# ictnlp/StreamSpeech

Hardware: AMD Instinct MI355X
Metric: real-time factor (RTFx = audio seconds / wall seconds) + utterances/sec, offline S2ST fr-en (higher is better)
Workload: dtype f32

## Files before the change

### include/streamspeech_hip.h

```cpp
#ifndef STREAMSPEECH_HIP_H
#define STREAMSPEECH_HIP_H

#include <stddef.h>
#include <stdint.h>

#ifdef __cplusplus
extern "C" {
#endif

#define SS_ABI_VERSION 2

typedef struct ss_model ss_model;
typedef struct ss_vocoder ss_vocoder;
typedef struct ss_scratch ss_scratch;
typedef struct ss_stream_pool ss_stream_pool;

typedef struct ss_config {
  int32_t input_feat, conv_channels, conv_kernel;
  int32_t enc_dim, enc_ffn, enc_heads, enc_layers, dw_kernel;
  int32_t src_vocab, tgt_vocab;
  int32_t mt_layers, dec_dim, dec_ffn, dec_heads;
  int32_t t2u_layers, unit_layers, unit_vocab, ctc_upsample;
  int32_t pad, eos, unk;
  int32_t max_rel_pos;
// ... 245 lines not shown
                             int64_t* h_n_samples);
int ss_batch_t2u_units_pad(ss_model* m, void* stream, int B, const float* d_feats, int feat_rows, const int32_t* h_n,
                           const int32_t* h_n_tail_pad, int t2u_causal, int mask_eos, int32_t* d_raw, int32_t* d_tokens,
                           int32_t* d_counts);
int ss_batch_mt_features(ss_model* m, void* stream, int B, const float* d_enc_out, const int32_t* h_Tp, const int32_t* h_tokens,
                         const int32_t* h_n_tokens, const int32_t* h_n_tail_pad, float* d_feats, int feat_rows);
int ss_batch_vocoder_tail(ss_vocoder* v, void* stream, int B, const int32_t* d_codes, const int32_t* h_K, const int32_t* h_n_new,
                          const int32_t* h_ctx, const int32_t* h_rf, int dur_prediction, float* d_out, int64_t out_capacity,
                          int32_t* h_win_first, int32_t* h_dur, int64_t* h_out_start, int64_t* h_n_out);

int ss_prof_enable(int cls_mask);
int ss_prof_enable_hi(int cls_mask);
int ss_prof_reset(void);
int ss_prof_read(int cls, double* h_ms_total, double* h_flops_total, int64_t* h_launches,
                 double* h_bytes_total);
int ss_prof_totals(int cls, double* h_flops_total, double* h_bytes_total, int64_t* h_launches);
int ss_prof_read_issued(int cls, double* h_issued_flops_total);
int ss_prof_shape_log(int on);
int ss_prof_shape_dump(char* buf, int cap);
int ss_prof_num_classes(void);
const char* ss_prof_class_name(int cls);

int ss_model_set_pack_invariant(ss_model* m, int on);
int ss_model_get_pack_invariant(ss_model* m);
int ss_debug_canon(int mode);

int ss_debug_last_logits(ss_model* m, void* stream, float* d_out, int64_t cap_floats, int* h_rows, int* h_cols);

int ss_op_ffn_fused(void* stream, const float* dX, int ldx, float* dY, int ldy, const float* ln_g, const float* ln_b,
                    const float* dW1, const float* db1, const float* dW2, const float* db2, float alpha,
                    const float* ln2_g, const float* ln2_b, int M, int D, int F);
int ss_debug_ffn(int grid, int row_tiles_per_wave, int enable);
int ss_debug_rtlin(int grid, int enable);
int ss_debug_conv_c64(int enable);
int ss_debug_conv_c32(int enable);
int ss_debug_conv_c16(int enable);
int64_t ss_debug_enc_step_launches(void);
int ss_op_ln_linear(void* stream, const float* dX, int ldx, const float* ln_g, const float* ln_b, const float* dW,
                    const float* dbias, const float* dR, int ldr, float* dC, int ldc, int M, int N, int K, int act, float alpha,
                    int glu);

int ss_debug_force_tile(int bm, int bn, int ks);
int ss_debug_sk_errors(void);
int ss_debug_attention_split(int v);
int ss_debug_attention_q16(int v);
int ss_debug_enc_step_inject_timeout(ss_model* m);
int ss_debug_scratch_audit(ss_scratch* sc, size_t* booked, size_t* held);
int ss_debug_mt_inject_timeout(ss_model* m);

int ss_op_conv_gemm(void* stream, const float* dA, int lda, const float* dW, const float* dbias,
                    const float* dR, int ldr, const float* dR2, int ldr2, float* dC, int ldc,
                    int M, int N, int Cin, int taps, int dil, int stride, int pad, int in_len,
                    int chunk, int in_act, float in_slope, int act, float alpha, float div, int glu);
int ss_op_conv_f16(void* stream, const float* dA, const float* dW, const float* dbias, const float* dR, const float* dR2,
                   float* dC, float* dC2, int M, int C, int taps, int dil, int in_act, float in_slope, int act, float div,
                   const int32_t* d_segs, int nseg);
int ss_op_layernorm(void* stream, const float* dx, int ldx, float* dy, int ldy, const float* dg,
                    const float* db, int M, int D, float eps);
int ss_op_attention(void* stream, const float* dQ, int ldq, const float* dK, int ldk, const float* dV,
                    int ldv, float* dO, int ldo, int Tq, int Tk, int H, float scale, int causal,
                    int chunk, const float* dP, int ldp, const float* du, const float* dv);
typedef struct ss_op_attn_args {
  const float* Q; const float* K; const float* V; float* O;
  int32_t ldq, ldk, ldv, ldo;
  int32_t Tq, Tk, H;
  float scale;
// ... 30 lines not shown
```

### streamspeech_amd/csrc/debug_ops.hip

```cpp
#include "model_internal.hpp"

extern "C" int ss_op_conv_gemm(void* stream, const float* dA, int lda, const float* dW, const float* dbias,
                               const float* dR, int ldr, const float* dR2, int ldr2, float* dC, int ldc, int M,
                               int N, int Cin, int taps, int dil, int stride, int pad, int in_len, int chunk,
                               int in_act, float in_slope, int act, float alpha, float div, int glu) {
  GemmArgs a;
  a.A = dA; a.lda = lda; a.W = dW; a.bias = dbias; a.R = dR; a.ldr = ldr; a.R2 = dR2; a.ldr2 = ldr2; a.C = dC; a.ldc = ldc;
  a.M = M; a.N = N; a.Cin = Cin; a.taps = taps; a.dil = dil; a.stride = stride; a.pad = pad; a.in_len = in_len;
  a.chunk = chunk; a.in_act = in_act; a.in_slope = in_slope; a.act = act; a.alpha = alpha; a.div = div; a.glu = glu;
  a.same_rows = (stride == 1 && M == in_len) ? 1 : 0;
  static thread_local std::map<hipStream_t, DevBuf> wino_tmps;
  DevBuf& wino_tmp = wino_tmps[(hipStream_t)stream];
  if ((conv_c64w_enabled() && N == 64 && Cin == 64 && taps >= 3 && conv_c64_eligible(a)) ||
      (conv_c128w_enabled() && N == 128 && Cin == 128 && taps >= 3 && a.same_rows && !glu) ||
      (conv_c256w_enabled() && N == 256 && Cin == 256 && taps >= 3 && a.same_rows && !glu) ||
      (conv_c32w_enabled() && N == 32 && Cin == 32 && taps >= 3 && conv_c32_eligible(a))) {
    RET(wino_tmp.ensure((size_t)N * ((taps + 2) / 3) * 4 * N * sizeof(float)));
    RET(launch_wino_pack(dW, wino_tmp.f(), N, taps, (hipStream_t)stream));
    a.Wwino = wino_tmp.f();
  }
  return launch_conv_gemm(a, (hipStream_t)stream);
}

extern "C" int ss_op_conv_f16(void* stream, const float* dA, const float* dW, const float* dbias, const float* dR, const float* dR2,
// ... 45 lines not shown
  return launch_conv_gemm(a, (hipStream_t)stream);
}
extern "C" int ss_debug_conv_c64(int enable) {
  if (enable == 4 || enable == 5) { conv_c64w_debug(enable == 5); return SS_OK; }
  if (enable == 6 || enable == 7) { conv_c128w_debug(enable == 7); return SS_OK; }
  if (enable == 8 || enable == 9) { conv_c256w_debug(enable == 9); return SS_OK; }
  conv_c64_debug(enable);
  return SS_OK;
}
extern "C" int ss_debug_conv_c32(int enable) {
  if (enable == 4 || enable == 5) { conv_c32w_debug(enable == 5); return SS_OK; }
  conv_c32_debug(enable);
  return SS_OK;
}
extern "C" int ss_debug_conv_c16(int enable) { conv_c16_debug(enable); return SS_OK; }
extern "C" int64_t ss_debug_enc_step_launches(void) { return (int64_t)enc_step_launch_count(); }
extern "C" int ss_debug_scratch_audit(ss_scratch* sc, size_t* booked, size_t* held) {
  if (!sc || !booked || !held) return SS_ERR_ARG;
  size_t sum = 0;
  bool foreign = false;
  for (DevBuf* b : sc->all()) {
    sum += b->bytes;
    if (b->acct != &sc->acct) foreign = true;
  }
  *booked = sc->acct.used;
  *held = sum;
  return foreign ? SS_ERR_ARG : SS_OK;
}
extern "C" int ss_debug_rtlin(int grid, int enable) {
  if (grid < 0) return SS_ERR_ARG;
  rtlin_debug(grid, enable);
  return SS_OK;
}
extern "C" int ss_debug_ffn(int grid, int row_tiles_per_wave, int enable) {
  if (grid < 0 || row_tiles_per_wave < -1 || row_tiles_per_wave > 4) return SS_ERR_ARG;
  ffn_fused_debug_grid(grid);
  ffn_fused_debug_rows(row_tiles_per_wave);
  if (enable >= 0) dispatch_edit([enable](Dispatch& d) { d.ffn_fusion = enable ? 1 : 0; });
  return SS_OK;
}

extern "C" int ss_op_layernorm(void* stream, const float* dx, int ldx, float* dy, int ldy, const float* dg,
                               const float* db, int M, int D, float eps) {
  return launch_layernorm(dx, ldx, dy, ldy, dg, db, M, D, eps, (hipStream_t)stream);
}

static int op_attn_bind_split(AttnArgs& a) {
  static void* scratch = nullptr;
  if (!scratch) {
    SS_HIP_CHECK(hipMalloc(&scratch, attention_split_bytes()));
    SS_HIP_CHECK(hipMemset(scratch, 0, attention_split_bytes()));
  }
  attention_bind_split(a, scratch);
  return SS_OK;
}

extern "C" int ss_op_attention(void* stream, const float* dQ, int ldq, const float* dK, int ldk, const float* dV,
                               int ldv, float* dO, int ldo, int Tq, int Tk, int H, float scale, int causal, int chunk,
                               const float* dP, int ldp, const float* du, const float* dv) {
  AttnArgs a;
  a.Q = dQ; a.ldq = ldq; a.K = dK; a.ldk = ldk; a.V = dV; a.ldv = ldv; a.O = dO; a.ldo = ldo;
  a.Tq = Tq; a.Tk = Tk; a.H = H; a.scale = scale; a.causal = causal; a.chunk = chunk;
  a.P = dP; a.ldp = ldp; a.bias_u = du; a.bias_v = dv;
  if (dP) RET(op_attn_bind_split(a));
  return launch_attention(a, (hipStream_t)stream);
}
// ... 70 lines not shown
```

### streamspeech_amd/csrc/dispatch.hpp

```cpp
#pragma once
#include <functional>

namespace ss {

struct Dispatch {
  int attn_no_mfma = 0;
  int attn_q16 = 1;
  int attn_split = 0;
  int c16_off = 0, c32_off = 0, c64_off = 0;
  long long c16_min_rows = 131072, c32_min_rows = 65536, c64_min_rows = 32768;
  int c64w_on = 1, c128w_on = 1, c256w_on = 1, c32w_on = 1;
  int c64w_min_k = 3;
  long long c128w_min_rows = 65536, c256w_min_rows = 32768;
  int sk_groups = 0;
  int ffn_force_g = 0;
  int ffn_wm = 3, ffn_wm_forced = 0;
  int ffn_fusion = 1;
  int ffn_min_rows = 1000;
  int force_bm = 0, force_bn = 0, force_ks = 0;
  double sk_min_flops = 4e9;
  int no_resblock_fusion = 0, no_pair_fusion = 0;
  int rt_off = 0, rt_min_rows = 193, rt_force_g = 0;
  long long rt_min_units = 4000;
  long long rt_kb_min_units = 256;
  int rt_kb_xmap = 1;
  int rt_kb_uw = 0;
};

const Dispatch& disp();
void dispatch_edit(const std::function<void(Dispatch&)>& fn);

struct CtxDispatch {
  Dispatch d;
  unsigned gen = 0xffffffffu;
  const Dispatch* refresh();
};
struct DispatchScope {
  explicit DispatchScope(const Dispatch* d);
  ~DispatchScope();
  const Dispatch* prev;
};

}
```

### streamspeech_amd/csrc/gemm.hip

```cpp
#include "gemm.hpp"

#include <atomic>
#include <cstdio>
#include <cstdlib>
#include <cstring>
#include <map>
#include <string>
#include <mutex>
#include <tuple>
#include <type_traits>
#include <utility>
#include <vector>

namespace ss {

using f32x4 = __attribute__((ext_vector_type(4))) float;

template <int BM, int BN, int BK, int WM, int WN, int KS, int PD, bool BLK = false>
__global__ __launch_bounds__(256 * KS) void conv_gemm_kernel(const GemmArgs p) {
  static_assert(WM * WN == 4, "4 waves per k-group");
  static_assert(!BLK || KS == 1, "the blocked chain is the KS = 1 form");
  constexpr int LDK = BK + 8;
  constexpr int WTM = BM / WM, WTN = BN / WN;
  constexpr int TM = WTM / 16, TN = WTN / 16;
  static_assert(TM >= 1 && TN >= 1, "wave tile must hold a 16x16 MFMA tile");
  constexpr int KQ = BK / 4;
  constexpr int A_F4 = BM * KQ, W_F4 = BN * KQ;
  constexpr int NA = (A_F4 + 255) / 256, NW = (W_F4 + 255) / 256;
  constexpr int STAGE = (BM + BN) * LDK;
  extern __shared__ __attribute__((aligned(16))) float smem_all[];
  const int kg = threadIdx.x >> 8;
  float* smem = smem_all + kg * 2 * STAGE;

  const int t = threadIdx.x & 255, lane = t & 63, wave = t >> 6;
  const int wm = wave / WN, wn = wave % WN;
  const int r = lane & 15, g = lane >> 4;

  int out_start = 0, out_len = p.M, in_start = 0, in_len = p.in_len, m_begin = p.m_begin, chunk = p.chunk;
  const float* A = p.A;
  if (p.nseg > 0) {
    const int* s = p.segs + 4 * blockIdx.z;
    out_start = s[0]; out_len = s[1]; in_start = s[2]; in_len = s[3];
    if (p.seg_mb) { m_begin = p.seg_mb[2 * blockIdx.z]; chunk = p.seg_mb[2 * blockIdx.z + 1]; }
    if (p.seg_A) A = p.seg_A[blockIdx.z];
  }
  const int m0 = blockIdx.x * BM + m_begin;
  if (m0 >= out_len) return;
  const int n0 = blockIdx.y * BN;
  const int kpt = p.Cin / BK;
// ... 265 lines not shown
          if (p.C2) p.C2[row * p.ldc2 + n + e] = x > 0.f ? x : x * p.c2_slope;
        }
      }
    }
  }
}


template <int SK, int WN, bool LNORM, bool GLU = false>
__global__ __launch_bounds__(256) void smallm_gemm_kernel(const GemmArgs p) {
  static_assert(SK * WN == 4, "4 waves");
  static_assert(!GLU || (SK == 2 && WN == 2), "GLU: wave column 0 = the 16 value columns, 1 = the 16 gate columns of a 32-column block");
  __shared__ f32x4 red[SK > 1 ? (SK - 1) * WN * 64 : 1];
  __shared__ float ln_stat[32];
  const int t = threadIdx.x, lane = t & 63, wave = t >> 6;
  const int sk = wave / WN, wn = wave % WN;
  const int r = lane & 15, g = lane >> 4;
  if ((int)blockIdx.x * (16 * WN) >= p.N) return;
  const int m0 = blockIdx.y * 16;
  const int n0 = blockIdx.x * (16 * WN) + wn * 16;
  const int K = p.Cin;
  const int KC = K / 16;
  const int c_begin = (KC * sk) / SK, c_end = (KC * (sk + 1)) / SK;

  const int am = m0 + r;
  const bool a_ok = am < p.M;
  const float* arow = p.A + (size_t)(a_ok ? am : 0) * p.lda + 4 * g;
  const int wnr = n0 + r;
  const bool w_ok = wnr < p.N;
  const float* wrow = p.W + (size_t)(w_ok ? wnr : 0) * K + 4 * g;

  float mean = 0.f, rstd = 1.f;
  if (LNORM) {
    const int lr = t >> 4, part = t & 15;
    const bool ok = (m0 + lr) < p.M;
    const float* xr = p.A + (size_t)(ok ? m0 + lr : 0) * p.lda + part * 4;
    f32x4 v[8];
    float sm = 0.f;
#pragma unroll
    for (int j = 0; j < 8; ++j) {
      v[j] = f32x4{0.f, 0.f, 0.f, 0.f};
      if (j * 64 < K && ok) v[j] = *reinterpret_cast<const f32x4*>(xr + j * 64);
      sm += (v[j][0] + v[j][1]) + (v[j][2] + v[j][3]);
    }
#pragma unroll
    for (int o = 1; o < 16; o <<= 1) sm += __shfl_xor(sm, o, 64);
    const float mu = sm / (float)K;
    float q = 0.f;
#pragma unroll
    for (int j = 0; j < 8; ++j)
      if (j * 64 < K) {
#pragma unroll
        for (int e = 0; e < 4; ++e) { const float d = v[j][e] - mu; q += d * d; }
      }
#pragma unroll
    for (int o = 1; o < 16; o <<= 1) q += __shfl_xor(q, o, 64);
    if (part == 0) { ln_stat[lr] = mu; ln_stat[16 + lr] = 1.0f / sqrtf(q / (float)K + 1e-5f); }
    __syncthreads();
    mean = ln_stat[r];
    rstd = ln_stat[16 + r];
  }

  f32x4 acc = {0.f, 0.f, 0.f, 0.f}, acc2 = {0.f, 0.f, 0.f, 0.f};
  f32x4 tot = {0.f, 0.f, 0.f, 0.f};
  const bool blocked = (c_end - c_begin) > 8;
  auto load4 = [&](f32x4 (&a)[4], f32x4 (&w)[4], int c) {
#pragma unroll
    for (int u = 0; u < 4; ++u) {
      a[u] = f32x4{0.f, 0.f, 0.f, 0.f};
      w[u] = f32x4{0.f, 0.f, 0.f, 0.f};
      if (a_ok) a[u] = *reinterpret_cast<const f32x4*>(arow + (c + u) * 16);
      if (w_ok) w[u] = *reinterpret_cast<const f32x4*>(wrow + (c + u) * 16);
    }
  };
  auto mma = [&](f32x4 a, f32x4 w, int c) {
    if (LNORM) {
      const f32x4 gm = *reinterpret_cast<const f32x4*>(p.ln_g + c * 16 + 4 * g);
      const f32x4 bt = *reinterpret_cast<const f32x4*>(p.ln_b + c * 16 + 4 * g);
#pragma unroll
      for (int e = 0; e < 4; ++e) a[e] = a_ok ? (a[e] - mean) * rstd * gm[e] + bt[e] : 0.f;
    }
    acc = __builtin_amdgcn_mfma_f32_16x16x4f32(a[0], w[0], acc, 0, 0, 0);
    acc2 = __builtin_amdgcn_mfma_f32_16x16x4f32(a[1], w[1], acc2, 0, 0, 0);
    acc = __builtin_amdgcn_mfma_f32_16x16x4f32(a[2], w[2], acc, 0, 0, 0);
    acc2 = __builtin_amdgcn_mfma_f32_16x16x4f32(a[3], w[3], acc2, 0, 0, 0);
    if (blocked && (c & 3) == 3) {
#pragma unroll
      for (int e = 0; e < 4; ++e) { tot[e] += acc[e] + acc2[e]; acc[e] = 0.f; acc2[e] = 0.f; }
    }
  };
  auto mma4 = [&](f32x4 (&a)[4], f32x4 (&w)[4], int c) {
#pragma unroll
    for (int u = 0; u < 4; ++u) mma(a[u], w[u], c + u);
  };
  const int G = (c_end - c_begin) / 4;
  f32x4 a0[4], w0[4], a1[4], w1[4];
  if (G > 0) load4(a0, w0, c_begin);
  for (int gi = 0; gi < G; gi += 2) {
    const int c = c_begin + 4 * gi;
    if (gi + 1 < G) load4(a1, w1, c + 4);
    mma4(a0, w0, c);
    if (gi + 1 < G) {
      if (gi + 2 < G) load4(a0, w0, c + 8);
      mma4(a1, w1, c + 4);
    }
  }
  for (int c = c_begin + 4 * G; c < c_end; ++c) {
    f32x4 a = {0.f, 0.f, 0.f, 0.f}, w = {0.f, 0.f, 0.f, 0.f};
    if (a_ok) a = *reinterpret_cast<const f32x4*>(arow + c * 16);
    if (w_ok) w = *reinterpret_cast<const f32x4*>(wrow + c * 16);
    mma(a, w, c);
  }
#pragma unroll
  for (int e = 0; e < 4; ++e) acc[e] = tot[e] + (acc[e] + acc2[e]);

  if (SK > 1) {
    if (sk > 0) red[((sk - 1) * WN + wn) * 64 + lane] = acc;
    __syncthreads();
    if (!GLU && sk > 0) return;
    if (sk == 0) {
#pragma unroll
      for (int s2 = 1; s2 < SK; ++s2) {
        const f32x4 o = red[((s2 - 1) * WN + wn) * 64 + lane];
#pragma unroll
        for (int e = 0; e < 4; ++e) acc[e] += o[e];
      }
    }
  }
  if constexpr (GLU) {
    __shared__ f32x4 gate_tile[64];
    const int ncol = n0 + r;
    const float bcol = (p.bias && ncol < p.N) ? p.bias[ncol] : 0.f;
    if (sk == 0 && wn == 1) {
      f32x4 gt;
#pragma unroll
      for (int e = 0; e < 4; ++e) gt[e] = acc[e] + bcol;
      gate_tile[lane] = gt;
    }
    __syncthreads();
    if (sk != 0 || wn != 0 || ncol + 16 >= p.N) return;
    const f32x4 gt = gate_tile[lane];
    const int oc = (int)blockIdx.x * 16 + r;
#pragma unroll
    for (int e = 0; e < 4; ++e) {
      const int m = m0 + g * 4 + e;
      if (m < p.M) p.C[(size_t)m * p.ldc + oc] = (acc[e] + bcol) * (1.0f / (1.0f + expf(-gt[e])));
    }
    return;
  }
  const int n = n0 + r;
  if (n >= p.N) return;
  const float b = p.bias ? p.bias[n] : 0.f;
#pragma unroll
  for (int e = 0; e < 4; ++e) {
    const int m = m0 + g * 4 + e;
    if (m < p.M) {
      float v = acc[e] + b;
      switch (p.act) {
        case ACT_SILU: v = v / (1.0f + expf(-v)); break;
        case ACT_RELU: v = fmaxf(v, 0.f); break;
        default: break;
      }
      v *= p.alpha;
      if (p.R) v += p.R[(size_t)m * p.ldr + n];
      p.C[(size_t)m * p.ldc + n] = v;
    }
  }
}


template <int MR, int KS, bool LNORM>
__global__ __launch_bounds__(256) void gemv_kernel(const GemmArgs p) {
  constexpr int WPB = 4;
  constexpr int CPB = WPB / KS;
  __shared__ float part[WPB][MR];
  const int t = threadIdx.x, lane = t & 63, wave = t >> 6;
  const int col = blockIdx.x * CPB + wave / KS;
  const int ks = wave % KS;
  const int K = p.Cin;
  const int kper = K / KS;
  const int k0 = ks * kper;
  const int nit = kper / 256;
  const bool col_ok = col < p.N;

  f32x4 wv[8];
  const float* wrow = p.W + (size_t)(col_ok ? col : 0) * K + k0 + 4 * lane;
#pragma unroll
  for (int it = 0; it < 8; ++it) {
    wv[it] = f32x4{0.f, 0.f, 0.f, 0.f};
    if (it < nit && col_ok) wv[it] = *reinterpret_cast<const f32x4*>(wrow + it * 256);
  }
  float acc[MR];
#pragma unroll
  for (int m = 0; m < MR; ++m) {
    acc[m] = 0.f;
    if (m >= p.M) continue;
    const float* xrow = p.A + (size_t)m * p.lda;
    float mean = 0.f, rstd = 1.f;
    if (LNORM) {
      f32x4 xv[8];
// ... 275 lines not shown
}
void sk_workspace_free(SkWorkspace* w) {
  if (!w) return;
  {
    std::lock_guard<std::mutex> lk(g_skw_mu);
    for (size_t i = 0; i < g_skw_live.size(); ++i)
      if (g_skw_live[i] == w) { g_skw_live.erase(g_skw_live.begin() + i); break; }
  }
  if (w->ws) (void)hipFree(w->ws);
  if (w->sync1) (void)hipFree(w->sync1);
  if (w->sync2) (void)hipFree(w->sync2);
  if (w->sync3) (void)hipFree(w->sync3);
  if (w->dbg) (void)hipFree(w->dbg);
  delete w;
}
namespace {
std::mutex g_disp_mu;
std::atomic<unsigned> g_disp_gen{1};
Dispatch env_defaults() {
  Dispatch d;
  auto I = [](const char* k, int dflt) { const char* e = getenv(k); return e ? atoi(e) : dflt; };
  auto L = [](const char* k, long long dflt) { const char* e = getenv(k); return e ? atoll(e) : dflt; };
  d.attn_split = I("SS_ATTN_NO_SPLIT", 0) ? -1 : 0; d.attn_q16 = I("SS_ATTN_Q16", d.attn_q16);
  d.c16_off = I("SS_NO_CONV_C16", 0) ? 1 : 0; d.c32_off = I("SS_NO_CONV_C32", 0) ? 1 : 0; d.c64_off = I("SS_NO_CONV_C64", 0) ? 1 : 0;
  d.c16_min_rows = L("SS_CONV_C16_MIN_ROWS", d.c16_min_rows); d.c32_min_rows = L("SS_CONV_C32_MIN_ROWS", d.c32_min_rows);
  d.c64_min_rows = L("SS_CONV_C64_MIN_ROWS", d.c64_min_rows);
  d.c64w_on = I("SS_CONV_C64_WINOGRAD", 1); d.c128w_on = I("SS_CONV_C128_WINOGRAD", 1); d.c256w_on = I("SS_CONV_C256_WINOGRAD", 1);
  d.c32w_on = I("SS_CONV_C32_WINOGRAD", 1); d.c64w_min_k = I("SS_CONV_C64_WINOGRAD_MIN_K", 3);
  d.c128w_min_rows = L("SS_CONV_C128_MIN_ROWS", d.c128w_min_rows); d.c256w_min_rows = L("SS_CONV_C256_MIN_ROWS", d.c256w_min_rows);
  if (getenv("SS_FFN_WM")) { d.ffn_wm = I("SS_FFN_WM", 3); d.ffn_wm_forced = 1; }
  d.ffn_fusion = I("SS_NO_FFN_FUSION", 0) ? 0 : 1; d.ffn_min_rows = I("SS_FFN_MIN_ROWS", d.ffn_min_rows);
  if (getenv("SS_SK_MIN_GFLOP")) d.sk_min_flops = 1e9 * atof(getenv("SS_SK_MIN_GFLOP"));
  d.no_resblock_fusion = I("SS_NO_RESBLOCK_FUSION", 0); d.no_pair_fusion = I("SS_NO_PAIR_FUSION", 0);
  d.rt_off = I("SS_NO_RTLIN", 0) ? 1 : 0; d.rt_min_rows = I("SS_RTLIN_MIN_ROWS", d.rt_min_rows); d.rt_min_units = L("SS_RTLIN_MIN_UNITS", d.rt_min_units);
  d.rt_kb_min_units = L("SS_RTLIN_KB_MIN_UNITS", d.rt_kb_min_units); d.rt_kb_uw = I("SS_RTLIN_KB_UW", d.rt_kb_uw); d.rt_kb_xmap = I("SS_RTLIN_KB_XMAP", d.rt_kb_xmap);
  return d;
}
Dispatch& process_settings() { static Dispatch d = env_defaults(); return d; }
thread_local const Dispatch* t_disp = nullptr;
thread_local CtxDispatch t_disp_own;
}
void dispatch_edit(const std::function<void(Dispatch&)>& fn) {
  std::lock_guard<std::mutex> lk(g_disp_mu);
  fn(process_settings());
  g_disp_gen.fetch_add(1, std::memory_order_release);
}
const Dispatch* CtxDispatch::refresh() {
  const unsigned now = g_disp_gen.load(std::memory_order_acquire);
  if (gen != now) {
    std::lock_guard<std::mutex> lk(g_disp_mu);
    d = process_settings();
    gen = g_disp_gen.load(std::memory_order_relaxed);
  }
  return &d;
}
const Dispatch& disp() { return t_disp ? *t_disp : *t_disp_own.refresh(); }
DispatchScope::DispatchScope(const Dispatch* d) : prev(t_disp) { t_disp = d; }
DispatchScope::~DispatchScope() { t_disp = prev; }

SkScope::SkScope(SkWorkspace* w) : prev(t_skw), prev_disp(t_disp) { t_skw = w; t_disp = w ? w->disp.refresh() : nullptr; }
SkScope::~SkScope() { t_skw = prev; t_disp = prev_disp; }

int sk_workspace_acquire(hipStream_t stream, SkWorkspace** out) {
  *out = nullptr;
  int dev = 0;
  SS_HIP_CHECK(hipGetDevice(&dev));
// ... 58 lines not shown
    for (unsigned* sy : {w->sync1, w->sync2}) {
      unsigned v = 0;
      if (sy && hipMemcpy(&v, sy + 8, sizeof(v), hipMemcpyDeviceToHost) == hipSuccess) total += (int)v;
    }
  return total;
}

void debug_force_tile(int bm, int bn, int ks) {
  dispatch_edit([=](Dispatch& d) { d.force_bm = bm; d.force_bn = bn; d.force_ks = ks; d.sk_groups = (bm == 1 && bn == 8); });
}
bool debug_tile_forced() { return disp().force_bm != 0; }

static thread_local int t_canon = CANON_NONE;
CanonScope::CanonScope(int mode) : prev(t_canon) { t_canon = mode; }
CanonScope::~CanonScope() { t_canon = prev; }
int canon_mode() { return t_canon; }
void canon_debug_set(int mode) { t_canon = mode; }

static bool smallm_shape_ok(const GemmArgs& a) {
  const bool glu_ok = !a.glu || (a.N % 32 == 0 && a.act == ACT_NONE && a.alpha == 1.f && !a.R);
  return a.taps == 1 && a.stride == 1 && a.pad == 0 && glu_ok && a.nseg == 0 && a.chunk == 0 && a.in_act == ACT_NONE && !a.R2 &&
         !a.C2 && a.div == 0.f && !a.ln_out && (a.act == ACT_NONE || a.act == ACT_SILU || a.act == ACT_RELU) && a.M > 0 &&
         a.M <= 1024 && a.Cin % 64 == 0 && (a.lda & 3) == 0 && (!a.ln_g || a.Cin <= 512);
}

static int launch_canon(const GemmArgs& a, hipStream_t stream) {
  const int M = a.nseg > 0 ? a.max_seg_out : a.M;
  const bool k32 = (a.Cin % 32) == 0;
  const int nseg = a.nseg > 0 ? a.nseg : 1;
  if (a.ln_out) return SS_ERR_ARG;
  if (a.canon == CANON_SMALLM) {
    if (!smallm_shape_ok(a)) return SS_ERR_ARG;
    if (a.glu) return launch_smallm<2, 2, true>(a, stream, PROF_SMALLM_2x2);
    if (a.Cin >= 1024 || a.N <= 4096) return launch_smallm<4, 1>(a, stream, PROF_SMALLM_4x1);
    return launch_smallm<2, 2>(a, stream, PROF_SMALLM_2x2);
  }
  if (a.seg_mb || a.seg_A) {
    if (a.nseg <= 0 || a.ln_g) return SS_ERR_ARG;
    return k32 ? launch_cfg<32, 64, 32, 2, 2, 1, 1, true>(a, stream, PROF_GEMM_32x64x32) : launch_cfg<32, 64, 16, 2, 2, 1, 1, true>(a, stream, PROF_GEMM_32x64x16);
  }
  if (rtlin_shape_ok(a) && (a.ln_g || rtlin_eligible(a))) return launch_rtlin(a, stream);
  if (a.ln_g) return SS_ERR_ARG;
  if (rtlin_kb_eligible(a)) return launch_rtlin_kb(a, stream);
  if (a.N <= 16) return launch_cfg<128, 16, 16, 4, 1, 1, 1, true>(a, stream, PROF_GEMM_128x16x16);
  if (a.N <= 32 && !a.glu) return k32 ? launch_cfg<128, 32, 32, 4, 1, 1, 1, true>(a, stream, PROF_GEMM_128x32x32) : launch_cfg<128, 32, 16, 4, 1, 1, 1, true>(a, stream, PROF_GEMM_128x32x16);
  if (M <= 16) return k32 ? launch_cfg<16, 128, 32, 1, 4, 1, 1, true>(a, stream, PROF_GEMM_16x128x32) : launch_cfg<16, 128, 16, 1, 4, 1, 1, true>(a, stream, PROF_GEMM_16x128x16);
  const long t3264 = (long)cdiv(M, 32) * cdiv(a.N, 64) * nseg;
  if (!k32) return launch_cfg<32, 64, 16, 2, 2, 1, 1, true>(a, stream, PROF_GEMM_32x64x16);
  if (a.glu || t3264 >= 768) return launch_cfg<32, 64, 32, 2, 2, 1, 1, true>(a, stream, PROF_GEMM_32x64x32);
  return launch_cfg<32, 32, 32, 2, 2, 1, 1, true>(a, stream, PROF_GEMM_32x32x32);
}

bool smallm_eligible(const GemmArgs& a) {
  if (disp().force_bm > 1) return false;
  const int M = a.nseg > 0 ? a.max_seg_out : a.M;
  const bool glu_ok = !a.glu || (a.N % 32 == 0 && a.act == ACT_NONE && a.alpha == 1.f && !a.R);
  const bool plain_linear = a.taps == 1 && a.stride == 1 && a.pad == 0 && glu_ok && a.nseg == 0 && a.chunk == 0 &&
                            a.in_act == ACT_NONE && !a.R2 && !a.C2 && a.div == 0.f &&
                            (a.act == ACT_NONE || a.act == ACT_SILU || a.act == ACT_RELU);
  static const int max_rows = getenv("SS_SMALLM_MAX_ROWS") ? atoi(getenv("SS_SMALLM_MAX_ROWS")) : 192;
  return plain_linear && M <= max_rows && M > 0 && a.Cin % 64 == 0 && (a.lda & 3) == 0;
}


int launch_conv_gemm(const GemmArgs& a_in, hipStream_t stream) {
  GemmArgs a = a_in;
// ... 86 lines not shown
```

### streamspeech_amd/csrc/gemm.hpp

```cpp
#pragma once
#include "common.hpp"
#include "dispatch.hpp"

namespace ss {

struct GemmArgs {
  const float* A = nullptr;
  const float* W = nullptr;
  const float* Wwino = nullptr;
  const void* Wf16 = nullptr;
  const float* bias = nullptr;
  const float* R = nullptr;
  const float* R2 = nullptr;
  float* C = nullptr;
  int lda = 0, ldc = 0, ldr = 0, ldr2 = 0;
  int M = 0, N = 0, Cin = 0;
  int taps = 1, dil = 1, stride = 1, pad = 0;
  int in_len = 0;
  int chunk = 0;
  int m_begin = 0;
  int in_act = ACT_NONE;
  float in_slope = 0.1f;
  int act = ACT_NONE;
  float alpha = 1.0f;
// ... 133 lines not shown
void conv_c64_debug(int enable);

bool conv_c32_eligible(const GemmArgs& a);
bool conv_c32_enabled();
int launch_conv_c32(const GemmArgs& a, hipStream_t stream);
void conv_c32_debug(int enable);

bool conv_c16_eligible(const GemmArgs& a);
bool conv_c16_enabled();
int launch_conv_c16(const GemmArgs& a, hipStream_t stream);
void conv_c16_debug(int enable);

bool conv_f16_eligible(const GemmArgs& a);
bool conv_f16_geometry_ok(int C, int taps, int dil);
int launch_conv_f16(const GemmArgs& a, hipStream_t stream);
size_t f16_pack_halves(int C, int taps);
int launch_f16_pack(const float* W, void* Wf, int C, int taps, hipStream_t stream);

bool rtlin_eligible(const GemmArgs& a);
bool rtlin_shape_ok(const GemmArgs& a);
int launch_rtlin(const GemmArgs& a, hipStream_t stream);
void rtlin_debug(int grid, int enable);
bool rtlin_kb_shape_ok(const GemmArgs& a);
bool rtlin_kb_eligible(const GemmArgs& a);
int launch_rtlin_kb(const GemmArgs& a, hipStream_t stream);

bool ffn_fused_eligible(int D, int F, int act, int M, int ldx, int ldy, bool canon = false);
int launch_ffn_fused(const float* X, int ldx, float* Y, int ldy, const float* ln_g, const float* ln_b, const float* W1,
                     const float* b1, const float* W2, const float* b2, float alpha, const float* ln2_g, const float* ln2_b,
                     int M, int D, int F, hipStream_t stream, int canon = 0);
void ffn_fused_debug_grid(int g);
void ffn_fused_debug_rows(int wm);

bool gemv_eligible(const GemmArgs& a);
bool smallm_eligible(const GemmArgs& a);

void debug_force_tile(int bm, int bn, int ks);
bool debug_tile_forced();

int launch_conv_gemm(const GemmArgs& a, hipStream_t stream);

}
```

### streamspeech_amd/lib.py

```python
import ctypes as C
import os

_HERE = os.path.dirname(os.path.abspath(__file__))
LIB_PATH = os.environ.get("SS_HIP_LIB") or os.path.join(_HERE, "libstreamspeech_hip.so")


class SSConfig(C.Structure):
    _fields_ = [(n, C.c_int32) for n in (
        "input_feat", "conv_channels", "conv_kernel", "enc_dim", "enc_ffn", "enc_heads", "enc_layers",
        "dw_kernel", "src_vocab", "tgt_vocab", "mt_layers", "dec_dim", "dec_ffn", "dec_heads",
        "t2u_layers", "unit_layers", "unit_vocab", "ctc_upsample", "pad", "eos", "unk",
        "max_rel_pos", "max_tgt_pos")]


class SSVocoderConfig(C.Structure):
    _fields_ = [
        ("num_embeddings", C.c_int32), ("embedding_dim", C.c_int32), ("model_in_dim", C.c_int32),
        ("upsample_initial_channel", C.c_int32),
        ("n_up", C.c_int32), ("upsample_rates", C.c_int32 * 8), ("upsample_kernel_sizes", C.c_int32 * 8),
        ("n_res", C.c_int32), ("resblock_kernel_sizes", C.c_int32 * 4), ("resblock_dilations", (C.c_int32 * 3) * 4),
        ("dur_hidden", C.c_int32), ("dur_kernel", C.c_int32)]


_vp, _i, _f, _i64 = C.c_void_p, C.c_int, C.c_float, C.c_int64
# ... 128 lines not shown
                                       C.POINTER(_f), C.POINTER(_f), _vp, _i]),
    "ss_batch_mt_beam_continue_plan": (_i, [_i, _i, C.POINTER(C.c_int32), C.POINTER(C.c_int32), C.POINTER(C.c_int32),
                                            C.POINTER(C.c_int32), _i, _i, _i, _i, _i, _i, _i, C.POINTER(C.c_int32),
                                            C.POINTER(C.c_int32), _i64, C.POINTER(_i64)]),
    "ss_batch_fbank_frames": (_i, [_vp, _vp, _i, C.POINTER(_vp), C.POINTER(C.c_int32), C.POINTER(C.c_int32), _f,
                                   C.POINTER(_vp)]),
    "ss_batch_fbank_frames_sr": (_i, [_vp, _vp, _i, C.POINTER(_vp), C.POINTER(C.c_int32), C.POINTER(C.c_int32), C.POINTER(C.c_int32),
                                      C.POINTER(_vp), C.POINTER(C.c_int32), C.POINTER(C.c_int32), C.POINTER(C.c_int32), _f,
                                      C.POINTER(_vp)]),
    "ss_fbank_sr_rows": (_i, [_i64, _i, _i, _i, C.POINTER(C.c_int32), C.POINTER(C.c_int32)]),
    "ss_batch_t2u_units": (_i, [_vp, _vp, _i, _vp, _i, C.POINTER(C.c_int32), _i, _i, _vp, _vp, _vp]),
    "ss_batch_vocoder_forward": (_i, [_vp, _vp, _i, _vp, C.POINTER(C.c_int32), _i, _vp, _vp, _i64, _vp,
                                      C.POINTER(_i64), C.POINTER(_i64)]),
    "ss_batch_t2u_units_pad": (_i, [_vp, _vp, _i, _vp, _i, C.POINTER(C.c_int32), C.POINTER(C.c_int32), _i, _i, _vp, _vp, _vp]),
    "ss_batch_mt_features": (_i, [_vp, _vp, _i, _vp, C.POINTER(C.c_int32), C.POINTER(C.c_int32), C.POINTER(C.c_int32),
                                  C.POINTER(C.c_int32), _vp, _i]),
    "ss_batch_vocoder_tail": (_i, [_vp, _vp, _i, _vp, C.POINTER(C.c_int32), C.POINTER(C.c_int32), C.POINTER(C.c_int32),
                                   C.POINTER(C.c_int32), _i, _vp, _i64, C.POINTER(C.c_int32), C.POINTER(C.c_int32),
                                   C.POINTER(_i64), C.POINTER(_i64)]),
    "ss_prof_enable": (_i, [_i]),
    "ss_prof_enable_hi": (_i, [_i]),
    "ss_prof_reset": (_i, []),
    "ss_prof_read": (_i, [_i, C.POINTER(C.c_double), C.POINTER(C.c_double), C.POINTER(_i64), C.POINTER(C.c_double)]),
    "ss_prof_totals": (_i, [_i, C.POINTER(C.c_double), C.POINTER(C.c_double), C.POINTER(_i64)]),
    "ss_prof_read_issued": (_i, [_i, C.POINTER(C.c_double)]),
    "ss_prof_shape_log": (_i, [_i]),
    "ss_prof_shape_dump": (_i, [C.c_char_p, _i]),
    "ss_prof_num_classes": (_i, []),
    "ss_prof_class_name": (C.c_char_p, [_i]),
    "ss_debug_force_tile": (_i, [_i, _i, _i]),
    "ss_op_ffn_fused": (_i, [_vp, _vp, _i, _vp, _i, _vp, _vp, _vp, _vp, _vp, _vp, _f, _vp, _vp, _i, _i, _i]),
    "ss_debug_ffn": (_i, [_i, _i, _i]),
    "ss_debug_rtlin": (_i, [_i, _i]),
    "ss_debug_conv_c64": (_i, [_i]),
    "ss_debug_conv_c32": (_i, [_i]),
    "ss_debug_conv_c16": (_i, [_i]),
    "ss_debug_enc_step_launches": (_i64, []),
    "ss_debug_scratch_audit": (_i, [_vp, C.POINTER(C.c_size_t), C.POINTER(C.c_size_t)]),
    "ss_op_ln_linear": (_i, [_vp, _vp, _i, _vp, _vp, _vp, _vp, _vp, _i, _vp, _i, _i, _i, _i, _i, _f, _i]),
    "ss_debug_last_logits": (_i, [_vp, _vp, _vp, _i64, C.POINTER(_i), C.POINTER(_i)]),
    "ss_debug_sk_errors": (_i, []),
    "ss_debug_attention_split": (_i, [_i]),
    "ss_debug_attention_q16": (_i, [_i]),
    "ss_op_conv_gemm": (_i, [_vp, _vp, _i, _vp, _vp, _vp, _i, _vp, _i, _vp, _i, _i, _i, _i, _i, _i, _i, _i, _i, _i,
                             _i, _f, _i, _f, _f, _i]),
    "ss_op_conv_f16": (_i, [_vp, _vp, _vp, _vp, _vp, _vp, _vp, _vp, _i, _i, _i, _i, _i, _f, _i, _f, _vp, _i]),
    "ss_op_layernorm": (_i, [_vp, _vp, _i, _vp, _i, _vp, _vp, _i, _i, _f]),
    "ss_op_attention": (_i, [_vp, _vp, _i, _vp, _i, _vp, _i, _vp, _i, _i, _i, _i, _f, _i, _i, _vp, _i, _vp, _vp]),
    "ss_op_attention_ex": (_i, [_vp, C.POINTER(SSOpAttnArgs)]),
    "ss_op_attention_pool": (_i, [_vp, C.POINTER(SSOpPoolAttnArgs)]),
    "ss_debug_attention_no_mfma": (_i, [_i]),
    "ss_op_dwconv_bn_silu": (_i, [_vp, _vp, _i, _vp, _i, _vp, _i, _vp, _vp, _vp, _vp, _f, _i, _i, _i]),
}

_lib = None


SS_ERR_ARG = 2
SS_ERR_CAPACITY = 4
SS_ERR_SCRATCH_CAP = 5
SS_ERR_STREAM_REPEAT = 8


class StreamSpeechHipError(RuntimeError):

    def __init__(self, msg, code=None):
# ... 32 lines not shown
```

Measured before the change: 6339.

## Add multi-tile decode-rows GEMM kernels for small-M linear layers

```diff
diff --git a/include/streamspeech_hip.h b/include/streamspeech_hip.h
--- a/include/streamspeech_hip.h
+++ b/include/streamspeech_hip.h
@@ -301,6 +301,7 @@
                     const float* ln2_g, const float* ln2_b, int M, int D, int F);
 int ss_debug_ffn(int grid, int row_tiles_per_wave, int enable);
 int ss_debug_rtlin(int grid, int enable);
+int ss_debug_decode_rows(int on);
 int ss_debug_conv_c64(int enable);
 int ss_debug_conv_c32(int enable);
 int ss_debug_conv_c16(int enable);
diff --git a/streamspeech_amd/csrc/debug_ops.hip b/streamspeech_amd/csrc/debug_ops.hip
--- a/streamspeech_amd/csrc/debug_ops.hip
+++ b/streamspeech_amd/csrc/debug_ops.hip
@@ -101,6 +101,11 @@
   rtlin_debug(grid, enable);
   return SS_OK;
 }
+extern "C" int ss_debug_decode_rows(int on) {
+  if (!decode_rows_form_ok(on)) return SS_ERR_ARG;
+  decode_rows_debug(on);
+  return SS_OK;
+}
 extern "C" int ss_debug_ffn(int grid, int row_tiles_per_wave, int enable) {
   if (grid < 0 || row_tiles_per_wave < -1 || row_tiles_per_wave > 4) return SS_ERR_ARG;
   ffn_fused_debug_grid(grid);
diff --git a/streamspeech_amd/csrc/decode_rows.hip b/streamspeech_amd/csrc/decode_rows.hip
--- /dev/null
+++ b/streamspeech_amd/csrc/decode_rows.hip
@@ -0,0 +1,281 @@
+#include "gemm.hpp"
+#include "smallm_common.hpp"
+
+namespace ss {
+
+template <int SK, int WN, bool LNORM, int MT, int NT>
+__global__ __launch_bounds__(256) void decode_rows_gemm_kernel(const GemmArgs p) {
+  static_assert(SK * WN == 4, "4 waves");
+  constexpr int TILES = MT * NT;
+  constexpr int CG = (MT + NT) <= 3 ? 4 : 2;
+  __shared__ f32x4 red[SK > 1 ? TILES * 4 * 64 : 1];
+  __shared__ float ln_stat[LNORM ? 32 * MT : 1];
+  const int t = threadIdx.x, lane = t & 63, wave = t >> 6;
+  const int sk = wave / WN, wn = wave % WN;
+  const int r = lane & 15, g = lane >> 4;
+  if ((int)blockIdx.x * (16 * WN * NT) >= p.N) return;
+  const int m0 = blockIdx.y * (16 * MT);
+  const int n0 = blockIdx.x * (16 * WN * NT) + wn * (16 * NT);
+  const int K = p.Cin;
+  const int KC = K / 16;
+  const int c_begin = (KC * sk) / SK, c_end = (KC * (sk + 1)) / SK;
+  const int mt = min(MT, (p.M - m0 + 15) / 16);
+
+  bool a_ok[MT], w_ok[NT];
+  const float* arow[MT];
+  const float* wrow[NT];
+#pragma unroll
+  for (int i = 0; i < MT; ++i) {
+    const int am = m0 + 16 * i + r;
+    a_ok[i] = am < p.M;
+    arow[i] = p.A + (size_t)(a_ok[i] ? am : 0) * p.lda + 4 * g;
+  }
+#pragma unroll
+  for (int j = 0; j < NT; ++j) {
+    const int wnr = n0 + 16 * j + r;
+    w_ok[j] = wnr < p.N;
+    wrow[j] = p.W + (size_t)(w_ok[j] ? wnr : 0) * K + 4 * g;
+  }
+
+  f32x4 acc[MT][NT], acc2[MT][NT], tot[MT][NT];
+#pragma unroll
+  for (int i = 0; i < MT; ++i)
+#pragma unroll
+    for (int j = 0; j < NT; ++j) acc[i][j] = acc2[i][j] = tot[i][j] = f32x4{0.f, 0.f, 0.f, 0.f};
+  const bool blocked = (c_end - c_begin) > 8;
+
+  auto load1 = [&](f32x4 (&a)[MT], f32x4 (&w)[NT], int c) {
+#pragma unroll
+    for (int i = 0; i < MT; ++i) {
+      a[i] = f32x4{0.f, 0.f, 0.f, 0.f};
+      if (i < mt && a_ok[i]) a[i] = *reinterpret_cast<const f32x4*>(arow[i] + c * 16);
+    }
+#pragma unroll
+    for (int j = 0; j < NT; ++j) {
+      w[j] = f32x4{0.f, 0.f, 0.f, 0.f};
+      if (w_ok[j]) w[j] = *reinterpret_cast<const f32x4*>(wrow[j] + c * 16);
+    }
+  };
+  float mean[MT], rstd[MT];
+#pragma unroll
+  for (int i = 0; i < MT; ++i) { mean[i] = 0.f; rstd[i] = 1.f; }
+  auto mma1 = [&](f32x4 (&a)[MT], f32x4 (&w)[NT], int c) {
+    f32x4 gm, bt;
+    if (LNORM) {
+      gm = *reinterpret_cast<const f32x4*>(p.ln_g + c * 16 + 4 * g);
+      bt = *reinterpret_cast<const f32x4*>(p.ln_b + c * 16 + 4 * g);
+    }
+    const bool flush = blocked && (c & 3) == 3;
+#pragma unroll
+    for (int i = 0; i < MT; ++i)
+      if (i < mt) {
+        const f32x4 an = LNORM ? smallm_ln_apply(a[i], a_ok[i], mean[i], rstd[i], gm, bt) : a[i];
+#pragma unroll
+        for (int j = 0; j < NT; ++j) smallm_chunk(an, w[j], acc[i][j], acc2[i][j], tot[i][j], flush);
+      }
+  };
+  auto loadg = [&](f32x4 (&a)[CG][MT], f32x4 (&w)[CG][NT], int c) {
+#pragma unroll
+    for (int u = 0; u < CG; ++u) load1(a[u], w[u], c + u);
+  };
+  auto mmag = [&](f32x4 (&a)[CG][MT], f32x4 (&w)[CG][NT], int c) {
+#pragma unroll
+    for (int u = 0; u < CG; ++u) mma1(a[u], w[u], c + u);
+  };
+  const int G = (c_end - c_begin) / CG;
+  f32x4 a0[CG][MT], w0[CG][NT], a1[CG][MT], w1[CG][NT];
+  if (G > 0) loadg(a0, w0, c_begin);
+  if (G > 1) loadg(a1, w1, c_begin + CG);
+  f32x4 rv[MT][NT];
+#pragma unroll
+  for (int i = 0; i < MT; ++i)
+#pragma unroll
+    for (int j = 0; j < NT; ++j) {
+      rv[i][j] = f32x4{0.f, 0.f, 0.f, 0.f};
+      const int n = n0 + 16 * j + r;
+      if (i < mt && n < p.N && (SK == 1 || (i * NT + j) % SK == sk)) rv[i][j] = smallm_residual(p, m0 + 16 * i + g * 4, n);
+    }
+  if (LNORM) {
+#pragma unroll
+    for (int i = 0; i < MT; ++i)
+      if (i < mt) smallm_ln_stats(p.A, p.lda, m0 + 16 * i, p.M, K, t, ln_stat + 32 * i);
+    __syncthreads();
+#pragma unroll
+    for (int i = 0; i < MT; ++i)
+      if (i < mt) { mean[i] = ln_stat[32 * i + r]; rstd[i] = ln_stat[32 * i + 16 + r]; }
+  }
+  for (int gi = 0; gi < G; gi += 2) {
+    const int c = c_begin + CG * gi;
+    mmag(a0, w0, c);
+    if (gi + 2 < G) loadg(a0, w0, c + 2 * CG);
+    if (gi + 1 < G) {
+      mmag(a1, w1, c + CG);
+      if (gi + 3 < G) loadg(a1, w1, c + 3 * CG);
+    }
+  }
+  if constexpr (CG > 1) {
+    for (int c = c_begin + CG * G; c < c_end; ++c) {
+      load1(a0[0], w0[0], c);
+      mma1(a0[0], w0[0], c);
+    }
+  }
+
+  if (SK > 1) {
+#pragma unroll
+    for (int i = 0; i < MT; ++i)
+#pragma unroll
+      for (int j = 0; j < NT; ++j)
+        if (i < mt) red[((i * NT + j) * 4 + wave) * 64 + lane] = smallm_range_result(acc[i][j], acc2[i][j], tot[i][j]);
+    __syncthreads();
+  }
+#pragma unroll
+  for (int i = 0; i < MT; ++i)
+#pragma unroll
+    for (int j = 0; j < NT; ++j) {
+      if (i >= mt) continue;
+      f32x4 v;
+      if (SK > 1) {
+        if ((i * NT + j) % SK != sk) continue;
+        v = red[((i * NT + j) * 4 + wn) * 64 + lane];
+#pragma unroll
+        for (int s2 = 1; s2 < SK; ++s2) {
+          const f32x4 o = red[((i * NT + j) * 4 + s2 * WN + wn) * 64 + lane];
+#pragma unroll
+          for (int e = 0; e < 4; ++e) v[e] += o[e];
+        }
+      } else {
+        v = smallm_range_result(acc[i][j], acc2[i][j], tot[i][j]);
+      }
+      const int n = n0 + 16 * j + r;
+      if (n < p.N) smallm_epilogue(p, v, m0 + 16 * i + g * 4, n, rv[i][j]);
+    }
+}
+
+constexpr int KB_MAX_BLOCKS = 32;
+template <int KW>
+__global__ __launch_bounds__(256 * KW) void decode_rows_kblock_kernel(const GemmArgs p) {
+  constexpr int SK = 4;
+  __shared__ f32x4 blk[KB_MAX_BLOCKS * 64];
+  const int t = threadIdx.x, lane = t & 63, wave = t >> 6;
+  const int r = lane & 15, g = lane >> 4;
+  if ((int)blockIdx.x * 16 >= p.N) return;
+  const int m0 = blockIdx.y * 16, n0 = blockIdx.x * 16;
+  const int K = p.Cin, KC = K / 16;
+  const int per_wave = KC / (SK * KW);
+  const int c0 = wave * per_wave;
+  const int am = m0 + r, wnr = n0 + r;
+  const bool a_ok = am < p.M, w_ok = wnr < p.N;
+  const float* arow = p.A + (size_t)(a_ok ? am : 0) * p.lda + 4 * g;
+  const float* wrow = p.W + (size_t)(w_ok ? wnr : 0) * K + 4 * g;
+  f32x4 rv = {0.f, 0.f, 0.f, 0.f};
+  for (int cb = 0; cb < per_wave; cb += 8) {
+    f32x4 a[8], w[8];
+#pragma unroll
+    for (int u = 0; u < 8; ++u) {
+      a[u] = f32x4{0.f, 0.f, 0.f, 0.f};
+      w[u] = f32x4{0.f, 0.f, 0.f, 0.f};
+      if (cb + u < per_wave) {
+        if (a_ok) a[u] = *reinterpret_cast<const f32x4*>(arow + (c0 + cb + u) * 16);
+        if (w_ok) w[u] = *reinterpret_cast<const f32x4*>(wrow + (c0 + cb + u) * 16);
+      }
+    }
+    if (cb == 0 && wave == 0 && wnr < p.N) rv = smallm_residual(p, m0 + g * 4, n0 + r);
+#pragma unroll
+    for (int b = 0; b < 2; ++b)
+      if (cb + 4 * b < per_wave) {
+        f32x4 acc = {0.f, 0.f, 0.f, 0.f}, acc2 = {0.f, 0.f, 0.f, 0.f}, s = {0.f, 0.f, 0.f, 0.f};
+#pragma unroll
+        for (int u = 0; u < 4; ++u) smallm_chunk(a[4 * b + u], w[4 * b + u], acc, acc2, s, u == 3);
+        blk[((c0 + cb) / 4 + b) * 64 + lane] = s;
+      }
+  }
+  __syncthreads();
+  if (wave != 0 || wnr >= p.N) return;
+  const int bpr = KC / (4 * SK);
+  f32x4 v;
+  const f32x4 zero = {0.f, 0.f, 0.f, 0.f};
+  for (int sk = 0; sk < SK; ++sk) {
+    f32x4 tot = {0.f, 0.f, 0.f, 0.f};
+    for (int b = 0; b < bpr; ++b) {
+      const f32x4 s = blk[(sk * bpr + b) * 64 + lane];
+#pragma unroll
+      for (int e = 0; e < 4; ++e) tot[e] += s[e];
+    }
+    const f32x4 o = smallm_range_result(zero, zero, tot);
+    if (sk == 0) v = o;
+    else {
+#pragma unroll
+      for (int e = 0; e < 4; ++e) v[e] += o[e];
+    }
+  }
+  smallm_epilogue(p, v, m0 + g * 4, n0 + r, rv);
+}
+
+static bool kblock_ok(const GemmArgs& a, int kw) {
+  const int KC = a.Cin / 16;
+  return !a.ln_g && !a.glu && (a.Cin >= 1024 || a.N <= 4096) &&
+         KC % (16 * kw) == 0 && KC / 4 > 8 && KC / 4 <= KB_MAX_BLOCKS;
+}
+
+template <int KW>
+static int launch_kblock(const GemmArgs& a, hipStream_t stream) {
+  dim3 grid((cdiv(a.N, 16) + 7) & ~7, cdiv(a.M, 16));
+  ProfRec rec{}; bool prof = false;
+  int rc = prof_begin(a, stream, PROF_SMALLM_4x1, rec, prof);
+  if (rc != SS_OK) return rc;
+  hipLaunchKernelGGL((decode_rows_kblock_kernel<KW>), grid, dim3(256 * KW), 0, stream, a);
+  SS_LAUNCH_CHECK();
+  return prof_end(stream, rec, prof);
+}
+
+template <int SK, int WN, int MT, int NT>
+static int launch_form(const GemmArgs& a, hipStream_t stream, ProfCls cls) {
+  dim3 grid((cdiv(a.N, 16 * WN * NT) + 7) & ~7, cdiv(a.M, 16 * MT));
+  ProfRec rec{}; bool prof = false;
+  int rc = prof_begin(a, stream, cls, rec, prof);
+  if (rc != SS_OK) return rc;
+  if (a.ln_g) hipLaunchKernelGGL((decode_rows_gemm_kernel<SK, WN, true, MT, NT>), grid, dim3(256), 0, stream, a);
+  else hipLaunchKernelGGL((decode_rows_gemm_kernel<SK, WN, false, MT, NT>), grid, dim3(256), 0, stream, a);
+  SS_LAUNCH_CHECK();
+  return prof_end(stream, rec, prof);
+}
+
+template <int SK, int WN>
+static int launch_sk(const GemmArgs& a, hipStream_t stream, ProfCls cls, int mt, int nt) {
+  switch (mt * 16 + nt) {
+    case 0x11: return launch_form<SK, WN, 1, 1>(a, stream, cls);
+    case 0x12: return launch_form<SK, WN, 1, 2>(a, stream, cls);
+    case 0x21: return launch_form<SK, WN, 2, 1>(a, stream, cls);
+    case 0x22: return launch_form<SK, WN, 2, 2>(a, stream, cls);
+    case 0x42: return launch_form<SK, WN, 4, 2>(a, stream, cls);
+    default: return SS_ERR_ARG;
+  }
+}
+
+void decode_rows_debug(int on) { dispatch_edit([on](Dispatch& d) { d.decode_rows = on; }); }
+
+bool decode_rows_form_ok(int on) {
+  if (on == 0 || on == 1) return true;
+  const int mt = (on >> 4) & 15, nt = on & 15;
+  if ((on >> 8) == 2) return on == 0x202 || on == 0x204;
+  return (on >> 8) == 1 && ((mt == 1 && (nt == 1 || nt == 2)) || (mt == 2 && (nt == 1 || nt == 2)) || (mt == 4 && nt == 2));
+}
+
+bool decode_rows_takes(const GemmArgs& a) {
+  return disp().decode_rows != 0 && !a.glu && a.M > 16 && (!a.ln_g || a.Cin <= 512);
+}
+
+int launch_decode_rows(const GemmArgs& a, hipStream_t stream) {
+  if (a.glu || a.M <= 0 || a.Cin % 64 != 0 || (a.lda & 3) != 0 || (a.ln_g && a.Cin > 512)) return SS_ERR_ARG;
+  const int on = disp().decode_rows;
+  if ((on >> 8) == 2 && kblock_ok(a, on & 15)) return (on & 15) == 4 ? launch_kblock<4>(a, stream) : launch_kblock<2>(a, stream);
+  if (on == 1 && kblock_ok(a, 4)) return launch_kblock<4>(a, stream);
+  const bool form41 = a.Cin >= 1024 || a.N <= 4096;
+  const long tiles = (long)cdiv(a.M, 16) * cdiv(a.N, form41 ? 16 : 32);
+  int mt = tiles > 800 ? 2 : 1, nt = mt;
+  if ((on >> 8) == 1) { mt = (on >> 4) & 15; nt = on & 15; }
+  if (form41) return launch_sk<4, 1>(a, stream, PROF_SMALLM_4x1, mt, nt);
+  return launch_sk<2, 2>(a, stream, PROF_SMALLM_2x2, mt, nt);
+}
+
+}
diff --git a/streamspeech_amd/csrc/dispatch.hpp b/streamspeech_amd/csrc/dispatch.hpp
--- a/streamspeech_amd/csrc/dispatch.hpp
+++ b/streamspeech_amd/csrc/dispatch.hpp
@@ -19,6 +19,7 @@
   int ffn_min_rows = 1000;
   int force_bm = 0, force_bn = 0, force_ks = 0;
   double sk_min_flops = 4e9;
+  int decode_rows = 1;
   int no_resblock_fusion = 0, no_pair_fusion = 0;
   int rt_off = 0, rt_min_rows = 193, rt_force_g = 0;
   long long rt_min_units = 4000;
diff --git a/streamspeech_amd/csrc/gemm.hip b/streamspeech_amd/csrc/gemm.hip
--- a/streamspeech_amd/csrc/gemm.hip
+++ b/streamspeech_amd/csrc/gemm.hip
@@ -1,4 +1,5 @@
 #include "gemm.hpp"
+#include "smallm_common.hpp"
 
 #include <atomic>
 #include <cstdio>
@@ -13,8 +14,6 @@
 #include <vector>
 
 namespace ss {
-
-using f32x4 = __attribute__((ext_vector_type(4))) float;
 
 template <int BM, int BN, int BK, int WM, int WN, int KS, int PD, bool BLK = false>
 __global__ __launch_bounds__(256 * KS) void conv_gemm_kernel(const GemmArgs p) {
@@ -346,30 +345,7 @@
 
   float mean = 0.f, rstd = 1.f;
   if (LNORM) {
-    const int lr = t >> 4, part = t & 15;
-    const bool ok = (m0 + lr) < p.M;
-    const float* xr = p.A + (size_t)(ok ? m0 + lr : 0) * p.lda + part * 4;
-    f32x4 v[8];
-    float sm = 0.f;
-#pragma unroll
-    for (int j = 0; j < 8; ++j) {
-      v[j] = f32x4{0.f, 0.f, 0.f, 0.f};
-      if (j * 64 < K && ok) v[j] = *reinterpret_cast<const f32x4*>(xr + j * 64);
-      sm += (v[j][0] + v[j][1]) + (v[j][2] + v[j][3]);
-    }
-#pragma unroll
-    for (int o = 1; o < 16; o <<= 1) sm += __shfl_xor(sm, o, 64);
-    const float mu = sm / (float)K;
-    float q = 0.f;
-#pragma unroll
-    for (int j = 0; j < 8; ++j)
-      if (j * 64 < K) {
-#pragma unroll
-        for (int e = 0; e < 4; ++e) { const float d = v[j][e] - mu; q += d * d; }
-      }
-#pragma unroll
-    for (int o = 1; o < 16; o <<= 1) q += __shfl_xor(q, o, 64);
-    if (part == 0) { ln_stat[lr] = mu; ln_stat[16 + lr] = 1.0f / sqrtf(q / (float)K + 1e-5f); }
+    smallm_ln_stats(p.A, p.lda, m0, p.M, K, t, ln_stat);
     __syncthreads();
     mean = ln_stat[r];
     rstd = ln_stat[16 + r];
@@ -391,17 +367,9 @@
     if (LNORM) {
       const f32x4 gm = *reinterpret_cast<const f32x4*>(p.ln_g + c * 16 + 4 * g);
       const f32x4 bt = *reinterpret_cast<const f32x4*>(p.ln_b + c * 16 + 4 * g);
-#pragma unroll
-      for (int e = 0; e < 4; ++e) a[e] = a_ok ? (a[e] - mean) * rstd * gm[e] + bt[e] : 0.f;
-    }
-    acc = __builtin_amdgcn_mfma_f32_16x16x4f32(a[0], w[0], acc, 0, 0, 0);
-    acc2 = __builtin_amdgcn_mfma_f32_16x16x4f32(a[1], w[1], acc2, 0, 0, 0);
-    acc = __builtin_amdgcn_mfma_f32_16x16x4f32(a[2], w[2], acc, 0, 0, 0);
-    acc2 = __builtin_amdgcn_mfma_f32_16x16x4f32(a[3], w[3], acc2, 0, 0, 0);
-    if (blocked && (c & 3) == 3) {
-#pragma unroll
-      for (int e = 0; e < 4; ++e) { tot[e] += acc[e] + acc2[e]; acc[e] = 0.f; acc2[e] = 0.f; }
-    }
+      a = smallm_ln_apply(a, a_ok, mean, rstd, gm, bt);
+    }
+    smallm_chunk(a, w, acc, acc2, tot, blocked && (c & 3) == 3);
   };
   auto mma4 = [&](f32x4 (&a)[4], f32x4 (&w)[4], int c) {
 #pragma unroll
@@ -425,8 +393,7 @@
     if (w_ok) w = *reinterpret_cast<const f32x4*>(wrow + c * 16);
     mma(a, w, c);
   }
-#pragma unroll
-  for (int e = 0; e < 4; ++e) acc[e] = tot[e] + (acc[e] + acc2[e]);
+  acc = smallm_range_result(acc, acc2, tot);
 
   if (SK > 1) {
     if (sk > 0) red[((sk - 1) * WN + wn) * 64 + lane] = acc;
@@ -464,22 +431,7 @@
   }
   const int n = n0 + r;
   if (n >= p.N) return;
-  const float b = p.bias ? p.bias[n] : 0.f;
-#pragma unroll
-  for (int e = 0; e < 4; ++e) {
-    const int m = m0 + g * 4 + e;
-    if (m < p.M) {
-      float v = acc[e] + b;
-      switch (p.act) {
-        case ACT_SILU: v = v / (1.0f + expf(-v)); break;
-        case ACT_RELU: v = fmaxf(v, 0.f); break;
-        default: break;
-      }
-      v *= p.alpha;
-      if (p.R) v += p.R[(size_t)m * p.ldr + n];
-      p.C[(size_t)m * p.ldc + n] = v;
-    }
-  }
+  smallm_epilogue(p, acc, m0 + g * 4, n, smallm_residual(p, m0 + g * 4, n));
 }
 
 
@@ -821,6 +773,7 @@
   d.ffn_fusion = I("SS_NO_FFN_FUSION", 0) ? 0 : 1; d.ffn_min_rows = I("SS_FFN_MIN_ROWS", d.ffn_min_rows);
   if (getenv("SS_SK_MIN_GFLOP")) d.sk_min_flops = 1e9 * atof(getenv("SS_SK_MIN_GFLOP"));
   d.no_resblock_fusion = I("SS_NO_RESBLOCK_FUSION", 0); d.no_pair_fusion = I("SS_NO_PAIR_FUSION", 0);
+  d.decode_rows = I("SS_NO_DECODE_ROWS", 0) ? 0 : 1;
   d.rt_off = I("SS_NO_RTLIN", 0) ? 1 : 0; d.rt_min_rows = I("SS_RTLIN_MIN_ROWS", d.rt_min_rows); d.rt_min_units = L("SS_RTLIN_MIN_UNITS", d.rt_min_units);
   d.rt_kb_min_units = L("SS_RTLIN_KB_MIN_UNITS", d.rt_kb_min_units); d.rt_kb_uw = I("SS_RTLIN_KB_UW", d.rt_kb_uw); d.rt_kb_xmap = I("SS_RTLIN_KB_XMAP", d.rt_kb_xmap);
   return d;
@@ -945,6 +898,7 @@
   if (a.canon == CANON_SMALLM) {
     if (!smallm_shape_ok(a)) return SS_ERR_ARG;
     if (a.glu) return launch_smallm<2, 2, true>(a, stream, PROF_SMALLM_2x2);
+    if (decode_rows_takes(a)) return launch_decode_rows(a, stream);
     if (a.Cin >= 1024 || a.N <= 4096) return launch_smallm<4, 1>(a, stream, PROF_SMALLM_4x1);
     return launch_smallm<2, 2>(a, stream, PROF_SMALLM_2x2);
   }
diff --git a/streamspeech_amd/csrc/gemm.hpp b/streamspeech_amd/csrc/gemm.hpp
--- a/streamspeech_amd/csrc/gemm.hpp
+++ b/streamspeech_amd/csrc/gemm.hpp
@@ -189,6 +189,11 @@
 void ffn_fused_debug_grid(int g);
 void ffn_fused_debug_rows(int wm);
 
+bool decode_rows_takes(const GemmArgs& a);
+int launch_decode_rows(const GemmArgs& a, hipStream_t stream);
+void decode_rows_debug(int on);
+bool decode_rows_form_ok(int on);
+
 bool gemv_eligible(const GemmArgs& a);
 bool smallm_eligible(const GemmArgs& a);
 
diff --git a/streamspeech_amd/csrc/smallm_common.hpp b/streamspeech_amd/csrc/smallm_common.hpp
--- /dev/null
+++ b/streamspeech_amd/csrc/smallm_common.hpp
@@ -0,0 +1,88 @@
+#pragma once
+#include "gemm.hpp"
+
+namespace ss {
+
+using f32x4 = __attribute__((ext_vector_type(4))) float;
+
+__device__ __forceinline__ void smallm_ln_stats(const float* A, int lda, int m0, int M, int K, int t, float* stat) {
+  const int lr = t >> 4, part = t & 15;
+  const bool ok = (m0 + lr) < M;
+  const float* xr = A + (size_t)(ok ? m0 + lr : 0) * lda + part * 4;
+  f32x4 v[8];
+  float sm = 0.f;
+#pragma unroll
+  for (int j = 0; j < 8; ++j) {
+    v[j] = f32x4{0.f, 0.f, 0.f, 0.f};
+    if (j * 64 < K && ok) v[j] = *reinterpret_cast<const f32x4*>(xr + j * 64);
+    sm += (v[j][0] + v[j][1]) + (v[j][2] + v[j][3]);
+  }
+#pragma unroll
+  for (int o = 1; o < 16; o <<= 1) sm += __shfl_xor(sm, o, 64);
+  const float mu = sm / (float)K;
+  float q = 0.f;
+#pragma unroll
+  for (int j = 0; j < 8; ++j)
+    if (j * 64 < K) {
+#pragma unroll
+      for (int e = 0; e < 4; ++e) { const float d = v[j][e] - mu; q += d * d; }
+    }
+#pragma unroll
+  for (int o = 1; o < 16; o <<= 1) q += __shfl_xor(q, o, 64);
+  if (part == 0) { stat[lr] = mu; stat[16 + lr] = 1.0f / sqrtf(q / (float)K + 1e-5f); }
+}
+
+__device__ __forceinline__ f32x4 smallm_ln_apply(f32x4 a, bool a_ok, float mean, float rstd, const f32x4& gm, const f32x4& bt) {
+#pragma unroll
+  for (int e = 0; e < 4; ++e) a[e] = a_ok ? (a[e] - mean) * rstd * gm[e] + bt[e] : 0.f;
+  return a;
+}
+
+__device__ __forceinline__ void smallm_chunk(const f32x4& a, const f32x4& w, f32x4& acc, f32x4& acc2, f32x4& tot, bool flush) {
+  acc = __builtin_amdgcn_mfma_f32_16x16x4f32(a[0], w[0], acc, 0, 0, 0);
+  acc2 = __builtin_amdgcn_mfma_f32_16x16x4f32(a[1], w[1], acc2, 0, 0, 0);
+  acc = __builtin_amdgcn_mfma_f32_16x16x4f32(a[2], w[2], acc, 0, 0, 0);
+  acc2 = __builtin_amdgcn_mfma_f32_16x16x4f32(a[3], w[3], acc2, 0, 0, 0);
+  if (flush) {
+#pragma unroll
+    for (int e = 0; e < 4; ++e) { tot[e] += acc[e] + acc2[e]; acc[e] = 0.f; acc2[e] = 0.f; }
+  }
+}
+
+__device__ __forceinline__ f32x4 smallm_range_result(const f32x4& acc, const f32x4& acc2, const f32x4& tot) {
+  f32x4 o;
+#pragma unroll
+  for (int e = 0; e < 4; ++e) o[e] = tot[e] + (acc[e] + acc2[e]);
+  return o;
+}
+
+__device__ __forceinline__ f32x4 smallm_residual(const GemmArgs& p, int m4, int n) {
+  f32x4 rv = {0.f, 0.f, 0.f, 0.f};
+  if (p.R) {
+#pragma unroll
+    for (int e = 0; e < 4; ++e)
+      if (m4 + e < p.M) rv[e] = p.R[(size_t)(m4 + e) * p.ldr + n];
+  }
+  return rv;
+}
+
+__device__ __forceinline__ void smallm_epilogue(const GemmArgs& p, const f32x4& acc, int m4, int n, const f32x4& rv) {
+  const float b = p.bias ? p.bias[n] : 0.f;
+#pragma unroll
+  for (int e = 0; e < 4; ++e) {
+    const int m = m4 + e;
+    if (m < p.M) {
+      float v = acc[e] + b;
+      switch (p.act) {
+        case ACT_SILU: v = v / (1.0f + expf(-v)); break;
+        case ACT_RELU: v = fmaxf(v, 0.f); break;
+        default: break;
+      }
+      v *= p.alpha;
+      if (p.R) v += rv[e];
+      p.C[(size_t)m * p.ldc + n] = v;
+    }
+  }
+}
+
+}
diff --git a/streamspeech_amd/lib.py b/streamspeech_amd/lib.py
--- a/streamspeech_amd/lib.py
+++ b/streamspeech_amd/lib.py
@@ -184,6 +184,7 @@
     "ss_op_ffn_fused": (_i, [_vp, _vp, _i, _vp, _i, _vp, _vp, _vp, _vp, _vp, _vp, _f, _vp, _vp, _i, _i, _i]),
     "ss_debug_ffn": (_i, [_i, _i, _i]),
     "ss_debug_rtlin": (_i, [_i, _i]),
+    "ss_debug_decode_rows": (_i, [_i]),
     "ss_debug_conv_c64": (_i, [_i]),
     "ss_debug_conv_c32": (_i, [_i]),
     "ss_debug_conv_c16": (_i, [_i]),
```

New measurement: 6291. Within noise of the previous version (-0.8%).
